# EndlessReform/smoltts

Measured on AMD Instinct MI355X. Metric: Mimi frames/sec (=12.5 x RTF), greedy DualAR decode + Mimi decode to PCM, higher is better.
Workload: dtype bf16 weights, fp32 activations/accumulate, fp32 KV cache (LM); fp32 (Mimi)

## Files before the change

smoltts_amd/csrc/argmax_dev.h:

```cpp
#pragma once
#include "x3.h"

namespace smoltts {

struct Top2 {
  float v1;
  int i1;
  float v2;
};
__device__ __forceinline__ Top2 top2_merge(Top2 a, Top2 b) {
  Top2 o;
  const bool a_first = (a.v1 > b.v1) || (a.v1 == b.v1 && a.i1 < b.i1);
  if (a_first) {
    o.v1 = a.v1; o.i1 = a.i1; o.v2 = fmaxf(a.v2, b.v1);
  } else {
    o.v1 = b.v1; o.i1 = b.i1; o.v2 = fmaxf(b.v2, a.v1);
  }
  return o;
}

__device__ __forceinline__ uint32_t mix32(uint32_t x) {
  x ^= x >> 16; x *= 0x7feb352dU; x ^= x >> 15; x *= 0x846ca68bU; x ^= x >> 16;
  return x;
}
__device__ __forceinline__ float uniform01(uint64_t seed, int slot, int frame, int step, int col) {
  uint32_t h = mix32((uint32_t)seed ^ 0x9E3779B9U * (uint32_t)(slot + 1));
  h = mix32(h ^ (uint32_t)(seed >> 32) ^ 0x85EBCA6BU * (uint32_t)(frame + 1));
  h = mix32(h ^ 0xC2B2AE35U * (uint32_t)(step + 1));
  h = mix32(h ^ 0x27D4EB2FU * (uint32_t)(col + 1));
  return ((float)(h >> 8) + 0.5f) * (1.0f / 16777216.0f);
}

struct ArgmaxScratch {
  Top2 sh[4];
  Top2 sh2[4];
  int id;
};

__device__ __forceinline__ int argmax_row(const float* row, int n_cols, bool ld_vec, int r, float* margin, const int* margin_mask,
                                          const SampleArgs& sa, ArgmaxScratch& S) {
  const int tid = threadIdx.x, lane = tid & 63, wave = tid >> 6;
  float temp = sa.temp, min_p = sa.min_p;
  uint64_t seed = sa.seed;
  int key_slot = r;
  if (sa.table) {
    const SmolttsSlotSampling en = sa.table[r];
    temp = sa.step == 0 ? en.temp : en.fast_temp;
    min_p = temp > 0.f ? en.min_p : 0.f;
    seed = en.seed;
    key_slot = 0;
  }
  Top2 t{-INFINITY, 0x7fffffff, -INFINITY};
#define ST_TAKE(V, J)                                                                               \
  {                                                                                                 \
    const float v_ = (V);                                                                           \
    if (v_ > t.v1) {  \
      t.v2 = t.v1; t.v1 = v_; t.i1 = (J);                                                           \
    } else if (v_ > t.v2) {                                                                         \
      t.v2 = v_;                                                                                    \
    }                                                                                               \
  }
  const bool vec = (n_cols & 3) == 0 && ld_vec && n_cols <= 8 * 1024;
  float4 v[8];
  if (vec) {
#pragma unroll
    for (int i = 0; i < 8; ++i) {
      const int j = tid * 4 + i * 1024;
      v[i] = j < n_cols ? *reinterpret_cast<const float4*>(row + j) : make_float4(-INFINITY, -INFINITY, -INFINITY, -INFINITY);
    }
#pragma unroll
    for (int i = 0; i < 8; ++i) {
      const int j = tid * 4 + i * 1024;
      if (j < n_cols) { ST_TAKE(v[i].x, j) ST_TAKE(v[i].y, j + 1) ST_TAKE(v[i].z, j + 2) ST_TAKE(v[i].w, j + 3) }
    }
  } else {
    for (int j = tid; j < n_cols; j += 256) ST_TAKE(row[j], j)
  }
#undef ST_TAKE
#pragma unroll
  for (int o = 32; o > 0; o >>= 1) {
    Top2 b;
    b.v1 = __shfl_xor(t.v1, o); b.i1 = __shfl_xor(t.i1, o); b.v2 = __shfl_xor(t.v2, o);
    t = top2_merge(t, b);
  }
  if (lane == 0) S.sh[wave] = t;
  __syncthreads();
  Top2 a = top2_merge(top2_merge(S.sh[0], S.sh[1]), top2_merge(S.sh[2], S.sh[3]));
  if (temp > 0.f) {
    const int frame = sa.frames ? sa.frames[r] : sa.frame_base + r;
    if (!sa.table && sa.salt) seed += 0x9E3779B97F4A7C15ULL * (uint64_t)sa.salt[r];
    const float inv_t = 1.0f / temp;
    const float cut = min_p > 0.f ? logf(min_p) : -INFINITY;
    Top2 k{-INFINITY, 0x7fffffff, -INFINITY};
#define ST_KEY(V, J)                                                  \
  {                                                                   \
    const float z = ((V) - a.v1) * inv_t;                   \
    if (z >= cut) {                                                   \
      const float u = uniform01(seed, key_slot, frame, sa.step, (J)); \
      const float key = z - logf(-logf(u));                           \
      if (key > k.v1) { k.v1 = key; k.i1 = (J); }                     \
    }                                                                 \
  }
    if (vec) {
#pragma unroll
      for (int i = 0; i < 8; ++i) {
        const int j = tid * 4 + i * 1024;
        if (j < n_cols) { ST_KEY(v[i].x, j) ST_KEY(v[i].y, j + 1) ST_KEY(v[i].z, j + 2) ST_KEY(v[i].w, j + 3) }
      }
    } else {
      for (int j = tid; j < n_cols; j += 256) ST_KEY(row[j], j)
    }
#undef ST_KEY
#pragma unroll
    for (int o = 32; o > 0; o >>= 1) {
      Top2 b;
      b.v1 = __shfl_xor(k.v1, o); b.i1 = __shfl_xor(k.i1, o); b.v2 = -INFINITY;
      k = top2_merge(k, b);
    }
    if (lane == 0) S.sh2[wave] = k;
    __syncthreads();
    const Top2 w = top2_merge(top2_merge(S.sh2[0], S.sh2[1]), top2_merge(S.sh2[2], S.sh2[3]));
    a.i1 = w.i1;
  }
  if (a.i1 < 0 || a.i1 >= n_cols) a.i1 = 0;
  if (tid == 0) {
    if (temp <= 0.f && margin && (margin_mask == nullptr || margin_mask[r])) {
      const float gap = a.v1 - a.v2;
      if (gap < margin[r]) {
        margin[r] = gap;
        if (sa.margin_at) sa.margin_at[r] = (sa.frames ? sa.frames[r] : sa.frame_base + r) * 64 + sa.step;
      }
    }
  }
  return a.i1;
}

template <int CTRL>
__device__ __forceinline__ Top2 top2_dpp(Top2 t) {
  Top2 b;
  b.v1 = __int_as_float(__builtin_amdgcn_update_dpp(0, __float_as_int(t.v1), CTRL, 0xF, 0xF, true));
  b.i1 = __builtin_amdgcn_update_dpp(0, t.i1, CTRL, 0xF, 0xF, true);
  b.v2 = __int_as_float(__builtin_amdgcn_update_dpp(0, __float_as_int(t.v2), CTRL, 0xF, 0xF, true));
  return top2_merge(t, b);
}
template <bool ROWS32>
__device__ __forceinline__ Top2 top2_swap(Top2 t, int lane) {
  const unsigned a[3] = {__float_as_uint(t.v1), (unsigned)t.i1, __float_as_uint(t.v2)};
  unsigned o[3];
  const bool upper = (lane & (ROWS32 ? 32 : 16)) != 0;
#pragma unroll
  for (int i = 0; i < 3; ++i) {
    if (ROWS32) {
      const auto r = __builtin_amdgcn_permlane32_swap(a[i], a[i], false, false);
      o[i] = upper ? r[0] : r[1];
    } else {
      const auto r = __builtin_amdgcn_permlane16_swap(a[i], a[i], false, false);
      o[i] = upper ? r[0] : r[1];
    }
  }
  return top2_merge(t, Top2{__uint_as_float(o[0]), (int)o[1], __uint_as_float(o[2])});
}
__device__ __forceinline__ Top2 cand_pick_wave(const float* cand, int tiles, int lane) {
  Top2 t{-INFINITY, 0x7fffffff, -INFINITY};
  for (int j = lane; j < tiles; j += 64) {
    const float4 c = *reinterpret_cast<const float4*>(cand + (size_t)j * 4);
    t = top2_merge(t, Top2{c.x, __float_as_int(c.y), c.z});
  }
  t = top2_dpp<0xB1>(t);
  t = top2_dpp<0x4E>(t);
  t = top2_dpp<0x141>(t);
  t = top2_dpp<0x140>(t);
  t = top2_swap<false>(t, lane);
  t = top2_swap<true>(t, lane);
  return t;
}

struct QkvGather {
  const float* table;
  const float* rope;
  float* q_out;
  float* kc;
  float* vc;
  int n_q_heads, n_kv_heads, cache_len, pos;
};

__device__ __forceinline__ float4 rope_gathered4(float4 v, float4 cs) {
#pragma clang fp contract(off)
  const float o0 = v.x * cs.x - v.y * cs.y, o1 = v.y * cs.x + v.x * cs.y;
  const float o2 = v.z * cs.z - v.w * cs.w, o3 = v.w * cs.z + v.z * cs.w;
  return make_float4(o0, o1, o2, o3);
}

constexpr int QG_MAX = 2;
struct QkvRegs { float4 v[QG_MAX], cs[QG_MAX]; };

__device__ __forceinline__ void qkv_gather_load(const QkvGather& g, long erow, int base, QkvRegs& o) {
  const int qd = g.n_q_heads * 64, kd = g.n_kv_heads * 64, nqkv = qd + 2 * kd;
  const float* trow = g.table + erow * nqkv;
#pragma unroll
  for (int i = 0; i < QG_MAX; ++i) {
    const int n0 = base + (threadIdx.x + i * 256) * 4;
    o.v[i] = n0 < nqkv ? *reinterpret_cast<const float4*>(trow + n0) : make_float4(0.f, 0.f, 0.f, 0.f);
    o.cs[i] = n0 < qd + kd ? *reinterpret_cast<const float4*>(g.rope + ((long)g.pos * 32 + ((n0 & 63) >> 1)) * 2) : make_float4(1.f, 0.f, 1.f, 0.f);
  }
}

__device__ __forceinline__ void qkv_gather_store(const QkvGather& g, int r, int base, const QkvRegs& in) {
  const int qd = g.n_q_heads * 64, kd = g.n_kv_heads * 64, nqkv = qd + 2 * kd;
#pragma unroll
  for (int i = 0; i < QG_MAX; ++i) {
    const int n0 = base + (threadIdx.x + i * 256) * 4;
    if (n0 >= nqkv) continue;
    float4 v = in.v[i];
    if (n0 < qd + kd) v = rope_gathered4(v, in.cs[i]);
    if (n0 < qd) {
      *reinterpret_cast<float4*>(g.q_out + (long)r * qd + n0) = v;
    } else {
      const int nn = n0 - qd;
      float* dst = nn < kd ? g.kc : g.vc;
      const int h = (nn < kd ? nn : nn - kd) >> 6, d = nn & 63;
      *reinterpret_cast<float4*>(dst + (((long)r * g.n_kv_heads + h) * g.cache_len + g.pos) * 64 + d) = v;
    }
  }
}

}
```

smoltts_amd/csrc/gemm3.hip:

```cpp
#include <stdlib.h>

#include "argmax_dev.h"
#ifndef SMOLTTS_DBG_PIECES
#define SMOLTTS_DBG_PIECES 3
#endif
#ifndef SMOLTTS_DBG_PIECES_RESID
#define SMOLTTS_DBG_PIECES_RESID SMOLTTS_DBG_PIECES
#endif

namespace smoltts {

struct Gemm3Dev {
  const char* w;
  const float* wscale;
  const char* x3;
  int M, N, K;
  int w_nt;
  int f8_act;
  int half_rows;
  const float* ssq_in;
  float eps;
  const float* bias;
  const float* resid;
  float* out;
// ... 585 lines not shown
  for (int g = 0; g < G; ++g) {
    const float* qp = PICK ? trow + (u.kvc * G + g) * 64 + 4 * m8 : p.aq + (long)row * qd + (u.kvc * G + g) * 64 + 4 * m8;
    u.qa[g] = *reinterpret_cast<const float4*>(qp);
    u.qb[g] = *reinterpret_cast<const float4*>(qp + 32);
  }
  if (PICK) {
    const float4 csa = *reinterpret_cast<const float4*>(p.pk_rope + ((long)p.a_pos * 32 + 2 * m8) * 2);
    const float4 csb = *reinterpret_cast<const float4*>(p.pk_rope + ((long)p.a_pos * 32 + 16 + 2 * m8) * 2);
#pragma unroll
    for (int g = 0; g < G; ++g) { u.qa[g] = rope_gathered4(u.qa[g], csa); u.qb[g] = rope_gathered4(u.qb[g], csb); }
    const float4 ra0 = rope_gathered4(u.ka0, csa), rb0 = rope_gathered4(u.kb0, csb);
    if (new0) { u.ka0 = ra0; u.kb0 = rb0; }
    if (TWO) {
      const float4 ra1 = rope_gathered4(u.ka1, csa), rb1 = rope_gathered4(u.kb1, csb);
      if (new1) { u.ka1 = ra1; u.kb1 = rb1; }
    }
    if (write_kv && u.hv && (new0 || new1)) {
      float* kw = p.kc + cb + (long)p.a_pos * 64;
      float* vw = p.vc + cb + (long)p.a_pos * 64;
      const float4 ka = new0 ? u.ka0 : u.ka1, kb = new0 ? u.kb0 : u.kb1, va = new0 ? u.va0 : u.va1, vb = new0 ? u.vb0 : u.vb1;
      *reinterpret_cast<float4*>(kw) = ka; *reinterpret_cast<float4*>(kw + 32) = kb;
      *reinterpret_cast<float4*>(vw + 32 * hb) = va; *reinterpret_cast<float4*>(vw + 32 * (1 - hb)) = vb;
    }
  }
}

template <int G, bool TWO>
__device__ __forceinline__ void awo_compute(const AwoUnit<G, TWO>& u, char* frag, int lane) {
#pragma clang fp contract(off)
  constexpr int R = AWO_R;
  const int hb = (lane >> 3) & 1, m8 = lane & 7;
  const bool up = (lane & 16) != 0;
#pragma unroll
  for (int g = 0; g < G; ++g) {
    const float4 a = make_float4(u.qa[g].x * 0.125f, u.qa[g].y * 0.125f, u.qa[g].z * 0.125f, u.qa[g].w * 0.125f);
    const float4 b = make_float4(u.qb[g].x * 0.125f, u.qb[g].y * 0.125f, u.qb[g].z * 0.125f, u.qb[g].w * 0.125f);
    float s0 = score16(a, b, u.ka0, u.kb0), s1 = -INFINITY;
    s0 = u.ok0 ? s0 : -INFINITY;
    if (TWO) {
      s1 = score16(a, b, u.ka1, u.kb1);
      s1 = u.ok1 ? s1 : -INFINITY;
    }
    float mx = TWO ? fmaxf(s0, s1) : s0;
    mx = fmaxf(mx, dpp_ror8(mx));
    {
      float t = mx;
      swap16(mx, t);
      mx = fmaxf(mx, t);
    }
    const float e0 = __expf(s0 - mx);
    float den = e0;
    float4 oa = make_float4(e0 * u.va0.x, e0 * u.va0.y, e0 * u.va0.z, e0 * u.va0.w);
    float4 ob = make_float4(e0 * u.vb0.x, e0 * u.vb0.y, e0 * u.vb0.z, e0 * u.vb0.w);
    if (TWO) {
      const float e1 = __expf(s1 - mx);
      den += e1;
      oa.x = fmaf(e1, u.va1.x, oa.x); oa.y = fmaf(e1, u.va1.y, oa.y); oa.z = fmaf(e1, u.va1.z, oa.z); oa.w = fmaf(e1, u.va1.w, oa.w);
      ob.x = fmaf(e1, u.vb1.x, ob.x); ob.y = fmaf(e1, u.vb1.y, ob.y); ob.z = fmaf(e1, u.vb1.z, ob.z); ob.w = fmaf(e1, u.vb1.w, ob.w);
    }
    den += dpp_ror8(den);
    {
      float t = den;
      swap16(den, t);
      den += t;
    }
    oa.x += dpp_ror8(ob.x); oa.y += dpp_ror8(ob.y); oa.z += dpp_ror8(ob.z); oa.w += dpp_ror8(ob.w);
    swap16(oa.x, oa.z);
    swap16(oa.y, oa.w);
    const float inv = 1.0f / den;
    const float ox = (oa.x + oa.z) * inv, oy = (oa.y + oa.w) * inv;
    uint32_t h, mm, l;
    split3_pair(ox, oy, h, mm, l);
    const int c = 2 * (u.kvc * G + g) + hb;
    char* fp = frag + ((size_t)((c * 3) * 4 + (m8 >> 1)) * R + u.rl) * 16 + (m8 & 1) * 8 + (up ? 4 : 0);
    if (u.hv) {
      *reinterpret_cast<uint32_t*>(fp) = h;
      *reinterpret_cast<uint32_t*>(fp + 4 * R * 16) = mm;
      *reinterpret_cast<uint32_t*>(fp + 8 * R * 16) = l;
    }
  }
}

constexpr int AWO_NA = 4, AWO_NB = 8, AWO_U = 3;

template <int G, int T, bool TWO, bool W8, bool PICK, int NBF>
__global__ __launch_bounds__(768) void attn_wo_kernel(const char* w_, const float* kc_, const float* vc_, const float* q_or_cand, const float* pk_table_,
                                                      int m_tiles, int N_, int K_, int heads_pos, Gemm3Dev p) {
  KernargTouch<AWO_KERNARG_LINES> kt;
  kernarg_touch(kt);
  p.w = w_; p.kc = const_cast<float*>(kc_); p.vc = const_cast<float*>(vc_); p.pk_table = pk_table_;
  if (PICK) p.pk_cand = q_or_cand; else p.aq = q_or_cand;
  p.M = m_tiles & 0xffff; p.pk_tiles = m_tiles >> 16; p.N = N_; p.K = K_;
  p.n_q_heads = heads_pos & 255; p.n_kv_heads = (heads_pos >> 8) & 255; p.cache_len = (heads_pos >> 16) & 255; p.a_pos = heads_pos >> 24;
  constexpr int WTILE = W8 ? 512 : 1024, WLANE = W8 ? 8 : 16;
  constexpr int R = AWO_R, NA = AWO_NA, NB = AWO_NB, U = AWO_U;
  extern __shared__ __attribute__((aligned(16))) float smem[];
  const int tid = threadIdx.x, wave = __builtin_amdgcn_readfirstlane(tid >> 6), lane = tid & 63;
  const int r = lane & 15, q = lane >> 4;
  const int ng = blockIdx.x, row0 = blockIdx.y * R;
  const int nchunks = p.K >> 5;
  constexpr bool FULL = NBF != 0;
  const int nb = FULL ? NBF : ((nchunks + 2) / 3 < 1 ? 1 : ((nchunks + 2) / 3 > NB ? NB : (nchunks + 2) / 3));
  char* frag = reinterpret_cast<char*>(smem);
  float4* red4 = reinterpret_cast<float4*>(frag + (size_t)nchunks * 3 * 4 * R * 16);
  STAMP3(0);

  if (wave < NA) {
    const int kv_pairs = (p.n_kv_heads + 1) >> 1;
    const int n_units = (p.M - row0 < R ? p.M - row0 : R) * kv_pairs;
    long erow0 = 0, erow1 = 0;
    Top2 t0{0.f, 0, 0.f}, t1 = t0;
#if SMOLTTS_DBG_AWO_ORDER
    if (PICK) __syncthreads();
#endif
    if (PICK) {
      const int n_cols = p.pk_tiles * 16;
      t0 = cand_pick_wave(p.pk_cand + (size_t)row0 * p.pk_tiles * 4, p.pk_tiles, lane);
      t1 = t0;
      if (row0 + 1 < p.M) t1 = cand_pick_wave(p.pk_cand + (size_t)(row0 + 1) * p.pk_tiles * 4, p.pk_tiles, lane);
      if (t0.i1 < 0 || t0.i1 >= n_cols) t0.i1 = 0;
      if (t1.i1 < 0 || t1.i1 >= n_cols) t1.i1 = 0;
      erow0 = (long)t0.i1 + p.pk_off;
      erow1 = (long)t1.i1 + p.pk_off;
    }
    AwoUnit<G, TWO> un;
    if (wave < n_units) awo_load<G, TWO, PICK>(un, p, wave, kv_pairs, row0, lane, wave / kv_pairs ? erow1 : erow0, blockIdx.x == 0);
    kernarg_touched(kt);
    const bool fin = wave < T;
    const int tf = fin ? wave : 0;
    const int m = row0 + r;
    const bool row_on = r < R;
    const bool mvalid = fin && row_on && m < p.M;
    float4 rr, bb, ga, gb, ws;
    rr = bb = make_float4(0.f, 0.f, 0.f, 0.f);
    ga = gb = ws = make_float4(1.f, 1.f, 1.f, 1.f);
    if (fin) {
      const int mc = m < p.M ? m : p.M - 1;
      const int n0r = (ng * T + tf) * 16 + q * 4;
      const int n0 = n0r < p.N ? n0r : p.N - 4;
      if (W8) ws = *reinterpret_cast<const float4*>(p.wscale + n0);
      if (PICK) {
        const uint2 e = *reinterpret_cast<const uint2*>(p.pk_emb + ((r & 1) ? erow1 : erow0) * p.K + n0);
        rr = make_float4(bf16_lo(e.x), bf16_hi(e.x), bf16_lo(e.y), bf16_hi(e.y));
      } else {
        rr = *reinterpret_cast<const float4*>(p.resid + (long)mc * p.ldo + n0);
      }
      if (p.bias != nullptr) bb = *reinterpret_cast<const float4*>(p.bias + n0);
      if (p.emit.x3a && p.emit.gamma_a) ga = *reinterpret_cast<const float4*>(p.emit.gamma_a + n0);
      if (p.emit.x3b && p.emit.gamma_b) gb = *reinterpret_cast<const float4*>(p.emit.gamma_b + n0);
    }
    STAMP3(5);
#if SMOLTTS_DBG_AWO_ORDER
    if (!PICK) __syncthreads();
#endif
    if (wave < n_units) awo_compute(un, frag, lane);
    for (int unit = wave + NA; unit < n_units; unit += NA) {
      awo_load<G, TWO, PICK>(un, p, unit, kv_pairs, row0, lane, unit / kv_pairs ? erow1 : erow0, blockIdx.x == 0);
      awo_compute(un, frag, lane);
    }
    STAMP3(6);
    __syncthreads();
    __syncthreads();
    STAMP3(3);
    if (PICK && blockIdx.x == 0 && wave == NA - 1 && lane == 0) {
#pragma unroll
      for (int rl = 0; rl < R; ++rl) {
        const int row = row0 + rl;
        if (row >= p.M) break;
        const Top2 t = rl ? t1 : t0;
        p.pk_ids[(long)row * p.pk_ids_stride] = t.i1;
        if (p.pk_margin && (p.pk_mask == nullptr || p.pk_mask[row])) {
          const float gap = t.v1 - t.v2;
          if (gap < p.pk_margin[row]) {
            p.pk_margin[row] = gap;
            if (p.pk_margin_at) p.pk_margin_at[row] = p.pk_frames[row] * 64 + p.pk_step;
          }
        }
      }
    }
    if (!fin) return;
    float4 part[NB];
#pragma unroll
    for (int w = 0; w < NB; ++w) part[w] = red4[((w < nb ? w : 0) * T + tf) * 64 + lane];
    float v[4] = {0.f, 0.f, 0.f, 0.f};
#pragma unroll
    for (int w = 0; w < NB; ++w) {
      const bool on = w < nb;
      v[0] += on ? part[w].x : 0.f;
      v[1] += on ? part[w].y : 0.f;
      v[2] += on ? part[w].z : 0.f;
      v[3] += on ? part[w].w : 0.f;
    }
    const int ntile = ng * T + tf;
    const int n0 = ntile * 16 + q * 4;
    const bool valid = mvalid && n0 < p.N;
    if (W8) { v[0] *= ws.x; v[1] *= ws.y; v[2] *= ws.z; v[3] *= ws.w; }
    v[0] = v[0] + bb.x + rr.x; v[1] = v[1] + bb.y + rr.y; v[2] = v[2] + bb.z + rr.z; v[3] = v[3] + bb.w + rr.w;
    if (valid) {
      *reinterpret_cast<float4*>(p.out + (long)m * p.ldo + n0) = make_float4(v[0], v[1], v[2], v[3]);
      if (p.emit.x3a) x3_emit4(p.emit.x3a, m, n0, p.N >> 5, v[0] * ga.x, v[1] * ga.y, v[2] * ga.z, v[3] * ga.w);
      if (p.emit.x3b) x3_emit4(p.emit.x3b, m, n0, p.N >> 5, v[0] * gb.x, v[1] * gb.y, v[2] * gb.z, v[3] * gb.w);
    }
    if (p.emit.ssq) {
      float sq = valid ? ((v[0] * v[0] + v[1] * v[1]) + (v[2] * v[2] + v[3] * v[3])) : 0.f;
      sq = sum_xor16_32(sq);
      if (q == 0 && mvalid && ntile * 16 < p.N) p.emit.ssq[(size_t)m * (p.N >> 4) + ntile] = sq;
    }
    STAMP3(4);
    return;
// ... 279 lines not shown
```

smoltts_amd/csrc/lm_engine.hip:

```cpp
#include <stdlib.h>
#include <string.h>

#include <new>

#include "argmax_dev.h"
#include "embed_dev.h"

using namespace smoltts;

struct SmolttsEngine {
  SmolttsLMConfig cfg;
  SmolttsLMWeights w;
  const char* arena;
  size_t arena_bytes;
  const float* fast_qkv;
};

constexpr int STAGE_RING = 8;

struct SmolttsSession {
  SmolttsEngine* e;
  int B, max_seq, max_rows, max_frames;
  int stop_on_eos;
  float temp, fast_temp, min_p;
// ... 118 lines not shown
  s->mask = cv.take<int>(B);
  s->iota = cv.take<int>(B);
  s->fastpos = cv.take<int>((size_t)c.n_fast * B);
  s->stage_slots = cv.take<int>(B);
  s->stage_last = cv.take<int>(B);
  s->margin = cv.take<float>(B);
  s->attn_part = cv.take<float>(ATT_SPLIT_PART_FLOATS);
  s->attn_ticket = cv.take<int>(ATT_SPLIT_MAX_PAIRS);
  s->margin_at = cv.take<int>(B);
  s->codes = cv.take<int>(B * (size_t)s->max_frames * H);
  s->slot_tab_area = cv.take<SmolttsSlotSampling>(2 * B + (B * sizeof(int) + sizeof(SmolttsSlotSampling) - 1) / sizeof(SmolttsSlotSampling));
  *total = cv.off;
}

__global__ void init_state_kernel(int B, int n_fast, int* iota, int* fastpos, int* pos, int* frames, int* done, int* mask,
                                  float* margin, int* margin_at, int* cur_col, int* new_col, int* salt, int* attn_ticket) {
  const int b = blockIdx.x * blockDim.x + threadIdx.x;
  for (int i = b; i < ATT_SPLIT_MAX_PAIRS; i += gridDim.x * blockDim.x) attn_ticket[i] = 0;
  if (b >= B) return;
  margin_at[b] = 0;
  iota[b] = b;
  for (int i = 0; i < n_fast; ++i) fastpos[i * B + b] = i;
  pos[b] = 0; frames[b] = 0; done[b] = 1; mask[b] = 0; salt[b] = 0;
  margin[b] = INFINITY;
  for (int i = 0; i <= n_fast; ++i) { cur_col[b * (1 + n_fast) + i] = 0; new_col[b * (1 + n_fast) + i] = 0; }
}

__global__ void slot_sampling_scatter_kernel(int n, const SmolttsSlotSampling* entries, const int* slots, SmolttsSlotSampling* table) {
  const int i = blockIdx.x * blockDim.x + threadIdx.x;
  if (i < n) table[slots[i]] = entries[i];
}

__global__ void slot_reset_kernel(int B, int n_slots, const int* slots, const int* last_row, const int* row_pos, int* pos,
                                  int* frames, int* done, int* mask, float* margin, int* salt) {
  const int b = blockIdx.x * blockDim.x + threadIdx.x;
  if (b >= B) return;
  int hit = -1;
  for (int i = 0; i < n_slots; ++i)
    if (slots[i] == b) hit = i;
  mask[b] = hit >= 0;
  if (hit >= 0) {
    pos[b] = row_pos[last_row[hit]] + 1;
    frames[b] = 0; done[b] = 0; margin[b] = INFINITY;
    salt[b] += 1;
  }
}

__global__ void slot_start_kernel(int B, int H, int n_slots, const int* slots, const int* last_row, const int* row_pos,
                                  const int* grid, int* pos, int* frames, int* done, float* margin, int* cur_col, int* salt) {
  const int b = blockIdx.x * blockDim.x + threadIdx.x;
  if (b >= B) return;
  for (int i = 0; i < n_slots; ++i)
    if (slots[i] == b) {
      const int lr = last_row[i];
      pos[b] = row_pos[lr];
      frames[b] = 0; done[b] = 0; margin[b] = INFINITY;
      salt[b] += 1;
      for (int k = 0; k < H; ++k) cur_col[b * H + k] = grid[(long)lr * H + k];
    }
}

__global__ void slot_park_kernel(int B, int n_slots, const int* slots, const int* last_row, const int* row_pos, int* pos,
                                 int* done, int* mask) {
  const int b = blockIdx.x * blockDim.x + threadIdx.x;
  if (b >= B) return;
  for (int i = 0; i < n_slots; ++i)
    if (slots[i] == b) { pos[b] = row_pos[last_row[i]] + 1; done[b] = 1; mask[b] = 0; }
}

__global__ void slot_parkpos_kernel(int B, int n_slots, const int* slots, const int* where, int* pos, int* done, int* mask) {
  const int b = blockIdx.x * blockDim.x + threadIdx.x;
  if (b >= B) return;
  for (int i = 0; i < n_slots; ++i)
    if (slots[i] == b) { pos[b] = where[i]; done[b] = 1; mask[b] = 0; }
}

struct CommitArgs {
  int B, H, max_frames, max_seq, im_end, stop_on_eos, advance_pos, do_commit;
  int* new_col;
  int *mask, *cur_col, *codes, *pos, *frames, *done;
  const float* slow_logits; int slow_cols; SampleArgs slow_sa;
  const float* last_logits; int last_cols; SampleArgs last_sa;
  float* margin;
  const float* slow_cand; int slow_tiles;
  const float* last_cand; int last_tiles;
  int* attn_ticket;
};

__global__ __launch_bounds__(256) void commit_embed_kernel(CommitArgs a, EmbedTables t, float* xt, EmitDev emit) {
  __shared__ int s_col[64];
  __shared__ float sh4[4];
  __shared__ ArgmaxScratch s_pick[2];
  const int b = blockIdx.x, tid = threadIdx.x, H = a.H;
  if (b == 0 && a.attn_ticket)
    for (int i = tid; i < ATT_SPLIT_MAX_PAIRS; i += blockDim.x) a.attn_ticket[i] = 0;
  int id_slow = 0, id_last = 0;
  const bool c_slow = a.slow_logits && a.slow_cand, c_last = a.last_logits && a.last_cand;
  if (c_slow || c_last) {
    __shared__ int s_id[2];
    __shared__ float s_gap[2];
    const int wave = tid >> 6, lane = tid & 63;
    if ((wave == 0 && c_slow) || (wave == 1 && c_last)) {
      const float* cand = wave == 0 ? a.slow_cand + (size_t)b * a.slow_tiles * 4 : a.last_cand + (size_t)b * a.last_tiles * 4;
      Top2 t = cand_pick_wave(cand, wave == 0 ? a.slow_tiles : a.last_tiles, lane);
      if (t.i1 < 0 || t.i1 >= (wave == 0 ? a.slow_cols : a.last_cols)) t.i1 = 0;
      if (lane == 0) { s_id[wave] = t.i1; s_gap[wave] = t.v1 - t.v2; }
    }
    __syncthreads();
    if (tid == 0 && a.margin && a.mask[b]) {
#pragma unroll
      for (int k = 0; k < 2; ++k) {
        if (!(k == 0 ? c_slow : c_last)) continue;
        const SampleArgs& sa = k == 0 ? a.slow_sa : a.last_sa;
        if (s_gap[k] < a.margin[b]) {
          a.margin[b] = s_gap[k];
          if (sa.margin_at) sa.margin_at[b] = (sa.frames ? sa.frames[b] : sa.frame_base + b) * 64 + sa.step;
        }
      }
    }
    if (c_slow) id_slow = s_id[0];
    if (c_last) id_last = s_id[1];
  }
  if (a.slow_logits && !c_slow) id_slow = argmax_row(a.slow_logits + (long)b * a.slow_cols, a.slow_cols, (a.slow_cols & 3) == 0, b, a.margin, a.mask, a.slow_sa, s_pick[0]);
  if (a.last_logits && !c_last) id_last = argmax_row(a.last_logits + (long)b * a.last_cols, a.last_cols, (a.last_cols & 3) == 0, b, a.margin, a.mask, a.last_sa, s_pick[1]);
  int f = 0;
  bool live = false;
  if (tid < 64) { f = a.frames[b]; live = a.do_commit && a.mask[b]; }
  const bool publish = live && f < a.max_frames;
  int slow_now = 0;
  if (tid < H) {
    int nv = a.new_col[b * H + tid];
    if (a.slow_logits && tid == 0) nv = id_slow;
    if (a.last_logits && tid == H - 1) nv = id_last;
    if ((a.slow_logits && tid == 0) || (a.last_logits && tid == H - 1)) a.new_col[b * H + tid] = nv;
    const int v = publish ? nv : a.cur_col[b * H + tid];
    s_col[tid] = v;
    if (publish) {
      a.cur_col[b * H + tid] = v;
      a.codes[((long)b * a.max_frames + f) * H + tid] = v;
    }
  }
  slow_now = a.slow_logits ? id_slow : a.new_col[b * H];
  if (tid == 0) {
    int d = a.done[b];
    if (live) {
      int p = a.pos[b];
      if (a.advance_pos) a.pos[b] = ++p;
      if (publish) a.frames[b] = f + 1;
      if ((a.stop_on_eos && slow_now == a.im_end) || f + 1 >= a.max_frames || p >= a.max_seq) a.done[b] = d = 1;
    }
    a.mask[b] = !d;
  }
  __syncthreads();
  embed_row(t, s_col, b, xt, emit, sh4);
}

SmolttsGemm3Args base3(int fmt, const void* w, const void* x3, int M, int N, int K, int epilogue) {
  SmolttsGemm3Args a;
  memset(&a, 0, sizeof(a));
  a.w_dev = w; a.x3_dev = x3; a.M = M; a.N = N; a.K = K; a.epilogue = epilogue;
  a.w_format = fmt;
  if (fmt == SMOLTTS_W_FP8) a.w_scale_dev = reinterpret_cast<const float*>(static_cast<const char*>(w) + (size_t)N * K);
  return a;
}

bool dup_hit(const SmolttsSession* s, int code, int N) { return s->dup_code == code && (s->dup_n <= 0 || s->dup_n == N); }

int launch_gemm3_m(const SmolttsSession* s, const SmolttsGemm3Args& a, hipStream_t st) {
  ST_TRY(launch_gemm3(a, st));
  if (a.epilogue != SMOLTTS_EPI_RESID && dup_hit(s, a.epilogue, a.N)) ST_TRY(launch_gemm3(a, st));
  return SMOLTTS_OK;
}

int run_block(const SmolttsSession* s, const SmolttsBlockWeights& bw, int dim, int n_head, int n_kv, int inter, float* x,
              float* q, int M, const int* row_pos, const int* row_slot, const float* rope, void* kc, void* vc,
              int cache_len, const char* in_x3, const EmitArgs& next, hipStream_t st, bool first_pos = false,
              int kv_format = SMOLTTS_KV_F32, int iota_pos = -1, bool qkv_done = false, int w_stream = 0,
              const SmolttsPickArgs* pick = nullptr) {
  const SmolttsEngine* e = s->e;
  const char* A = e->arena;
  const float eps = e->cfg.norm_eps;
  if (!qkv_done) {
    SmolttsGemm3Args a = base3(e->cfg.weight_format, A + bw.wqkv, in_x3, M, (n_head + 2 * n_kv) * 64, dim, SMOLTTS_EPI_QKV_ROPE);
    a.fp8_activations = s->fp8_prefill;
    a.ssq_in_dev = s->ssq; a.eps = eps; a.out_dev = q; a.ldo = n_head * 64;
    a.rope_dev = rope; a.row_pos_dev = row_pos; a.row_slot_dev = row_slot;
    a.k_cache_dev = (float*)kc; a.v_cache_dev = (float*)vc; a.n_q_heads = n_head; a.n_kv_heads = n_kv; a.cache_len = cache_len;
    a.kv_format = kv_format; a.w_stream = (w_stream & (1 | SMOLTTS_STREAM_W_DEPTH_QKVO)) != 0;
    if (first_pos) a.v_x3_dev = s->x3a;
    ST_TRY(launch_gemm3_m(s, a, st));
  }
  const bool fused_attn = !first_pos && iota_pos > 0 && s->fuse_depth_attn && kv_format == SMOLTTS_KV_F32 &&
                          smoltts_gemm3_attn_fusable(n_head, n_kv, cache_len) && dim == n_head * 64;
  if (!first_pos && !fused_attn) {
    const int reps = dup_hit(s, cache_len <= 16 ? 100 : 101, 0) ? 2 : 1;
    for (int i = 0; i < reps; ++i)
      ST_TRY(launch_attention(q, kc, vc, row_pos, row_slot, M, n_head, n_kv, cache_len, 0, nullptr, s->x3a, st, kv_format, iota_pos,
                              s->split_attn ? s->attn_part : nullptr, s->attn_ticket));
  }
  {
    SmolttsGemm3Args a = base3(e->cfg.weight_format, A + bw.wo, s->x3a, M, dim, dim, SMOLTTS_EPI_RESID);
    a.fp8_activations = s->fp8_prefill;
    a.resid_dev = x; a.out_dev = x; a.ldo = dim;
    a.emit_a_dev = s->x3n; a.gamma_a_dev = (const float*)(A + bw.ffn_norm); a.ssq_out_dev = s->ssq; a.w_stream = (w_stream & (1 | SMOLTTS_STREAM_W_DEPTH_QKVO)) != 0;
    if (fused_attn) {
      a.attn_q_dev = q; a.attn_pos = iota_pos; a.k_cache_dev = (float*)kc; a.v_cache_dev = (float*)vc;
      a.n_q_heads = n_head; a.n_kv_heads = n_kv; a.cache_len = cache_len; a.kv_format = SMOLTTS_KV_F32;
      a.pick = pick;
    }
    ST_REQUIRE(pick == nullptr || fused_attn, SMOLTTS_E_STATE, "run_block: a pick needs the fused depth attention");
    ST_TRY(launch_gemm3(a, st));
  }
  {
    SmolttsGemm3Args a = base3(e->cfg.weight_format, A + bw.w13, s->x3n, M, 2 * inter, dim, SMOLTTS_EPI_SWIGLU);
    a.fp8_activations = s->fp8_prefill;
    a.ssq_in_dev = s->ssq; a.eps = eps; a.x3_out_dev = s->x3h; a.w_stream = (w_stream & (1 | SMOLTTS_STREAM_W_DEPTH_W13)) != 0;
    ST_TRY(launch_gemm3_m(s, a, st));
  }
  {
    SmolttsGemm3Args a = base3(e->cfg.weight_format, A + bw.w2, s->x3h, M, dim, inter, SMOLTTS_EPI_RESID);
    a.fp8_activations = s->fp8_prefill;
    a.resid_dev = x; a.out_dev = x; a.ldo = dim;
    a.emit_a_dev = next.x3a; a.gamma_a_dev = next.gamma_a; a.emit_b_dev = next.x3b; a.gamma_b_dev = next.gamma_b;
    a.ssq_out_dev = next.ssq; a.w_stream = (w_stream & (1 | SMOLTTS_STREAM_W_DEPTH_W2)) != 0;
    ST_TRY(launch_gemm3(a, st));
  }
  return SMOLTTS_OK;
}

const float* gamma_at(const SmolttsEngine* e, uint64_t off) { return (const float*)(e->arena + off); }

EmitArgs slow_hidden_emit(const SmolttsSession* s) {
  const SmolttsEngine* e = s->e;
  EmitArgs em{s->x3n, gamma_at(e, e->w.norm), s->x3n2,
              e->cfg.has_fast_project_in ? nullptr : gamma_at(e, e->w.fast_layers[0].attn_norm), s->ssq};
  return em;
}

__global__ __launch_bounds__(256) void scatter_last_kernel(const float* xr, const int* slots, const int* last_row, int dim,
                                                           float* xt) {
  const int i = blockIdx.x;
  const long src = last_row[i], dst = slots[i];
  for (int d = threadIdx.x * 4; d < dim; d += 256 * 4)
    *reinterpret_cast<float4*>(xt + dst * dim + d) = *reinterpret_cast<const float4*>(xr + src * dim + d);
}

EmbedTables embed_tables(const SmolttsEngine* e) {
  const SmolttsLMConfig& c = e->cfg;
  const char* A = e->arena;
  return EmbedTables{(const uint16_t*)(A + e->w.text_emb), (const uint16_t*)(A + e->w.codebook_emb), c.dim, c.codebook_size,
                     c.duplicate_code_0 ? 0 : c.codebook_size, c.embed_mask_mode, c.semantic_start_id, c.semantic_end_id,
                     c.vocab_size, c.codebook_size * c.num_codebooks, c.n_fast};
}

bool slow_sampled(const SmolttsSession* s) { return s->slot_mode ? (s->form & 1) != 0 : s->temp > 0.f; }
bool fast_sampled(const SmolttsSession* s) { return s->slot_mode ? (s->form & 2) != 0 : s->fast_temp > 0.f; }

SampleArgs pick_args(const SmolttsSession* s, int step) {
  if (s->slot_mode) {
    const bool sampled = step == 0 ? slow_sampled(s) : fast_sampled(s);
    return SampleArgs{0.f, 0.f, 0, step, 0, s->frames, nullptr, s->margin_at, sampled ? s->slot_tab : nullptr};
  }
  if (step == 0) return SampleArgs{s->temp, s->min_p, s->seed, 0, 0, s->frames, s->salt, s->margin_at, nullptr};
  return SampleArgs{s->fast_temp, s->fast_temp > 0.f ? s->min_p : 0.f, s->seed, step, 0, s->frames, s->salt, s->margin_at, nullptr};
}

bool commit_cand_slow(const SmolttsSession* s) { return s->commit_picks && s->fuse_pick && !slow_sampled(s) && s->B < 256; }
bool commit_cand_last(const SmolttsSession* s) { return s->commit_picks && s->fuse_pick && !fast_sampled(s) && s->B < 256; }

int launch_commit_embed(SmolttsSession* s, int do_commit, int advance_pos, hipStream_t st, bool picks = false) {
  const SmolttsEngine* e = s->e;
  const SmolttsLMConfig& c = e->cfg;
  ST_REQUIRE(1 + c.n_fast <= 64 && c.dim % 64 == 0, SMOLTTS_E_INVALID, "commit: grid height > 64 or dim %% 64 != 0");
  CommitArgs a;
  memset(&a, 0, sizeof(a));
  a.B = s->B; a.H = 1 + c.n_fast; a.max_frames = s->max_frames; a.max_seq = s->max_seq; a.im_end = c.im_end_id;
  a.stop_on_eos = s->stop_on_eos; a.advance_pos = advance_pos; a.do_commit = do_commit;
  a.new_col = s->new_col; a.mask = s->mask; a.cur_col = s->cur_col; a.codes = s->codes; a.pos = s->pos; a.frames = s->frames; a.done = s->done;
  a.margin = s->margin;
  a.attn_ticket = s->attn_ticket;
  if (picks) {
    a.slow_logits = s->logits_slow; a.slow_cols = c.vocab_size;
    a.slow_sa = pick_args(s, 0);
    a.last_logits = s->logits; a.last_cols = c.codebook_size;
    a.last_sa = pick_args(s, c.n_fast);
    if (commit_cand_slow(s)) { a.slow_cand = s->cand_slow; a.slow_tiles = (c.vocab_size + 15) / 16; }
    if (commit_cand_last(s)) { a.last_cand = s->cand; a.last_tiles = (c.codebook_size + 15) / 16; }
  }
  const EmitDev em{s->x3n, gamma_at(e, e->w.layers[0].attn_norm), nullptr, nullptr, s->ssq};
  hipLaunchKernelGGL(commit_embed_kernel, dim3(s->B), dim3(256), 0, st, a, embed_tables(e), s->xt, em);
  ST_CHECK_HIP(hipGetLastError());
  return SMOLTTS_OK;
}

int run_tail(SmolttsSession* s, int advance_pos, hipStream_t st) {
  const SmolttsEngine* e = s->e;
  const SmolttsLMConfig& c = e->cfg;
  const char* A = e->arena;
  const int B = s->B, H = 1 + c.n_fast;
  {
    SmolttsGemm3Args a = base3(c.weight_format, A + e->w.head, s->x3n, B, c.vocab_size, c.dim, SMOLTTS_EPI_STORE);
    a.ssq_in_dev = s->ssq; a.eps = c.norm_eps; a.out_dev = s->logits_slow; a.ldo = c.vocab_size; a.w_stream = (s->stream_w & SMOLTTS_STREAM_W_SLOW_HEAD) != 0;
    if (commit_cand_slow(s)) a.cand_out_dev = s->cand_slow;
    ST_TRY(launch_gemm3_m(s, a, st));
  }
  const bool picks = s->commit_picks;
  if (!picks) {
    const SampleArgs slow_sa = pick_args(s, 0);
    ST_TRY(launch_argmax(s->logits_slow, B, c.vocab_size, c.vocab_size, s->new_col, H, s->margin, s->mask, nullptr, 0, 0, nullptr,
                         nullptr, &slow_sa, st));
  }
  float* xf = s->xt;
  const char* first_x3 = s->x3n2;
  const EmitArgs to_fast0{s->x3n, gamma_at(e, e->w.fast_layers[0].attn_norm), nullptr, nullptr, s->ssq};
  if (c.has_fast_project_in) {
    SmolttsGemm3Args a = base3(c.weight_format, A + e->w.fast_proj_w, s->x3n2, B, c.fast_dim, c.dim, SMOLTTS_EPI_STORE);
    a.bias_dev = (const float*)(A + e->w.fast_proj_b); a.out_dev = s->xf; a.ldo = c.fast_dim;
    a.emit_a_dev = to_fast0.x3a; a.gamma_a_dev = to_fast0.gamma_a; a.ssq_out_dev = s->ssq;
    ST_TRY(launch_gemm3(a, st));
    xf = s->xf;
    first_x3 = s->x3n;
  }
  const size_t fl_stride = (size_t)B * c.fast_n_kv_head * c.n_fast * 64;
  const bool table = e->fast_qkv != nullptr && s->use_qkv_table;
  const bool pick_fused = s->fuse_pick && table && s->fuse_depth_attn && !fast_sampled(s) && B < 256 && c.codebook_size % 16 == 0 &&
                          c.fast_dim == c.fast_n_head * 64 && smoltts_gemm3_attn_fusable(c.fast_n_head, c.fast_n_kv_head, c.n_fast);
  SmolttsPickArgs pk;
  memset(&pk, 0, sizeof(pk));
  bool pk_pending = false;
  for (int i = 0; i < c.n_fast; ++i) {
    for (int l = 0; l < c.n_fast_layer; ++l) {
      const EmitArgs next{s->x3n,
                          gamma_at(e, l + 1 < c.n_fast_layer ? e->w.fast_layers[l + 1].attn_norm : e->w.fast_norm),
                          nullptr, nullptr, s->ssq};
      ST_TRY(run_block(s, e->w.fast_layers[l], c.fast_dim, c.fast_n_head, c.fast_n_kv_head, c.fast_inter, xf, s->qt, B,
                       s->fastpos + (size_t)i * B, s->iota, (const float*)(A + e->w.fast_rope), s->fkc + l * fl_stride,
                       s->fvc + l * fl_stride, c.n_fast, (i == 0 && l == 0) ? first_x3 : s->x3n, next, st, i == 0,
                       SMOLTTS_KV_F32, i, table && i > 0 && l == 0,
                       s->stream_w & (SMOLTTS_STREAM_W_DEPTH_QKVO | SMOLTTS_STREAM_W_DEPTH_W13 | SMOLTTS_STREAM_W_DEPTH_W2),
                       (pk_pending && l == 0) ? &pk : nullptr));
      if (l == 0) pk_pending = false;
    }
    {
      const size_t wrow = (size_t)i * e->w.fast_head_step_stride;
      const size_t wbytes = c.weight_format == SMOLTTS_W_FP8 ? wrow * (c.fast_dim + 4) : wrow * c.fast_dim * 2;
      SmolttsGemm3Args a = base3(c.weight_format, A + e->w.fast_head + wbytes, s->x3n, B, c.codebook_size, c.fast_dim, SMOLTTS_EPI_STORE);
      a.ssq_in_dev = s->ssq; a.eps = c.norm_eps; a.out_dev = s->logits; a.ldo = c.codebook_size;
      a.w_stream = (s->stream_w & SMOLTTS_STREAM_W_DEPTH_HEAD) != 0;
      if (pick_fused && i + 1 < c.n_fast) a.cand_out_dev = s->cand;
      if (i + 1 == c.n_fast && commit_cand_last(s)) a.cand_out_dev = s->cand;
      ST_TRY(launch_gemm3_m(s, a, st));
    }
    const SampleArgs fast_sa = pick_args(s, 1 + i);
    if (i + 1 == c.n_fast) {
      if (!picks)
        ST_TRY(launch_argmax(s->logits, B, c.codebook_size, c.codebook_size, s->new_col + 1 + i, H, s->margin, s->mask, nullptr, 0, 0,
                             nullptr, nullptr, &fast_sa, st));
      break;
    }
    const int off = c.depthwise_wte ? (c.duplicate_code_0 ? i : i + 1) * c.codebook_size : 0;
    float* xnext = c.has_fast_project_in ? s->xf : s->xt;
    if (pick_fused) {
      pk.cand_dev = s->cand; pk.cand_tiles = c.codebook_size / 16; pk.qkv_table_dev = e->fast_qkv;
      pk.rope_dev = (const float*)(A + e->w.fast_rope); pk.emb_dev = A + e->w.fast_emb; pk.emb_row_offset = off;
      pk.ids_dev = s->new_col + 1 + i; pk.ids_stride = H; pk.margin_dev = s->margin; pk.margin_mask_dev = s->mask;
      pk.margin_at_dev = s->margin_at; pk.frames_dev = s->frames; pk.step = 1 + i;
      pk_pending = true;
      xf = xnext;
      continue;
    }
    QkvGather qg;
    memset(&qg, 0, sizeof(qg));
    if (table)
// ... 668 lines not shown
```

smoltts_amd/csrc/x3.h:

```cpp
#pragma once
#include "common.h"

namespace smoltts {

typedef __bf16 bf16x2_t __attribute__((ext_vector_type(2)));
typedef __bf16 bf16x8_t __attribute__((ext_vector_type(8)));

__device__ __forceinline__ uint32_t pack_bf16(float a, float b) {
  bf16x2_t h = {(__bf16)a, (__bf16)b};
  return __builtin_bit_cast(uint32_t, h);
}

__device__ __forceinline__ void split3_pair(float a, float b, uint32_t& h, uint32_t& m, uint32_t& l) {
  h = pack_bf16(a, b);
  const float ra = a - bf16_lo(h), rb = b - bf16_hi(h);
  m = pack_bf16(ra, rb);
  l = pack_bf16(ra - bf16_lo(m), rb - bf16_hi(m));
}

__device__ __forceinline__ size_t x3_offset(int m, int k, int nchunks) {
  const int mtile = m >> 4, r = m & 15, c = k >> 5, q = (k & 31) >> 3, j0 = k & 7;
  return ((size_t)mtile * nchunks + c) * 3072 + (size_t)(q * 16 + r) * 16 + j0 * 2;
}

__device__ __forceinline__ void x3_emit4(char* x3, int m, int k, int nchunks, float a0, float a1, float a2, float a3) {
  uint32_t h0, m0, l0, h1, m1, l1;
  split3_pair(a0, a1, h0, m0, l0);
  split3_pair(a2, a3, h1, m1, l1);
  char* p = x3 + x3_offset(m, k, nchunks);
  *reinterpret_cast<uint2*>(p) = make_uint2(h0, h1);
  *reinterpret_cast<uint2*>(p + 1024) = make_uint2(m0, m1);
  *reinterpret_cast<uint2*>(p + 2048) = make_uint2(l0, l1);
}

__device__ __forceinline__ void x3_emit2(char* x3, int m, int k, int nchunks, float a0, float a1) {
  uint32_t h, mm, l;
  split3_pair(a0, a1, h, mm, l);
  char* p = x3 + x3_offset(m, k, nchunks);
  *reinterpret_cast<uint32_t*>(p) = h;
  *reinterpret_cast<uint32_t*>(p + 1024) = mm;
  *reinterpret_cast<uint32_t*>(p + 2048) = l;
}

struct EmitDev {
  char* x3a;
  const float* gamma_a;
  char* x3b;
  const float* gamma_b;
  float* ssq;
};

__device__ __forceinline__ void emit_x4(const EmitDev& e, int m, int k, int nchunks, float x0, float x1, float x2, float x3v) {
  if (e.x3a) {
    if (e.gamma_a) {
      const float4 g = *reinterpret_cast<const float4*>(e.gamma_a + k);
      x3_emit4(e.x3a, m, k, nchunks, x0 * g.x, x1 * g.y, x2 * g.z, x3v * g.w);
    } else {
      x3_emit4(e.x3a, m, k, nchunks, x0, x1, x2, x3v);
    }
  }
  if (e.x3b) {
    if (e.gamma_b) {
      const float4 g = *reinterpret_cast<const float4*>(e.gamma_b + k);
      x3_emit4(e.x3b, m, k, nchunks, x0 * g.x, x1 * g.y, x2 * g.z, x3v * g.w);
    } else {
      x3_emit4(e.x3b, m, k, nchunks, x0, x1, x2, x3v);
    }
  }
}

__device__ __forceinline__ void emit_row_ssq(const EmitDev& e, int m, int dim, float local_ss, float* sh4) {
  if (!e.ssq) return;
  const int lane = threadIdx.x & 63, wave = threadIdx.x >> 6;
  float s = local_ss;
#pragma unroll
  for (int o = 32; o > 0; o >>= 1) s += __shfl_xor(s, o);
  if (lane == 0) sh4[wave] = s;
  __syncthreads();
  const int nt = dim >> 4;
  for (int i = threadIdx.x; i < nt; i += blockDim.x)
    e.ssq[(size_t)m * nt + i] = i == 0 ? ((sh4[0] + sh4[1]) + sh4[2]) + sh4[3] : 0.f;
}

}
```

Measured before the change: 28650.

## Batch candidate loads, overlap pick with attention load, specialize commit kernel

Candidate top-2 picks now load all tiles into registers with unrolled, predicated loads instead of a strided loop. In the attention+wo kernel, each wave computes its own row's pick first and issues its weight/KV load before merging the other row, so the load overlaps the second merge. The commit kernel is templated on whether row argmax is needed and takes candidate pointers as direct kernargs with prefetch, moving the ticket reset after the pick. It also switches shuffles to a lane_xor_c helper and makes top2_merge branch-free. The changes add code size and template variants.

```diff
diff --git a/smoltts_amd/csrc/argmax_dev.h b/smoltts_amd/csrc/argmax_dev.h
--- a/smoltts_amd/csrc/argmax_dev.h
+++ b/smoltts_amd/csrc/argmax_dev.h
@@ -1,5 +1,9 @@
 #pragma once
 #include "x3.h"
+
+#ifndef SMOLTTS_OPT_PICK_LOADS
+#define SMOLTTS_OPT_PICK_LOADS 1
+#endif
 
 namespace smoltts {
 
@@ -9,14 +13,9 @@
   float v2;
 };
 __device__ __forceinline__ Top2 top2_merge(Top2 a, Top2 b) {
-  Top2 o;
-  const bool a_first = (a.v1 > b.v1) || (a.v1 == b.v1 && a.i1 < b.i1);
-  if (a_first) {
-    o.v1 = a.v1; o.i1 = a.i1; o.v2 = fmaxf(a.v2, b.v1);
-  } else {
-    o.v1 = b.v1; o.i1 = b.i1; o.v2 = fmaxf(b.v2, a.v1);
-  }
-  return o;
+  const bool a_first = (a.v1 > b.v1) | ((a.v1 == b.v1) & (a.i1 < b.i1));
+  const float va2 = fmaxf(a.v2, b.v1), vb2 = fmaxf(b.v2, a.v1);
+  return Top2{a_first ? a.v1 : b.v1, a_first ? a.i1 : b.i1, a_first ? va2 : vb2};
 }
 
 __device__ __forceinline__ uint32_t mix32(uint32_t x) {
@@ -80,7 +79,7 @@
 #pragma unroll
   for (int o = 32; o > 0; o >>= 1) {
     Top2 b;
-    b.v1 = __shfl_xor(t.v1, o); b.i1 = __shfl_xor(t.i1, o); b.v2 = __shfl_xor(t.v2, o);
+    b.v1 = lane_xor_c(t.v1, o, lane); b.i1 = __float_as_int(lane_xor_c(__int_as_float(t.i1), o, lane)); b.v2 = lane_xor_c(t.v2, o, lane);
     t = top2_merge(t, b);
   }
   if (lane == 0) S.sh[wave] = t;
@@ -114,7 +113,7 @@
 #pragma unroll
     for (int o = 32; o > 0; o >>= 1) {
       Top2 b;
-      b.v1 = __shfl_xor(k.v1, o); b.i1 = __shfl_xor(k.i1, o); b.v2 = -INFINITY;
+      b.v1 = lane_xor_c(k.v1, o, lane); b.i1 = __float_as_int(lane_xor_c(__int_as_float(k.i1), o, lane)); b.v2 = -INFINITY;
       k = top2_merge(k, b);
     }
     if (lane == 0) S.sh2[wave] = k;
@@ -160,12 +159,7 @@
   }
   return top2_merge(t, Top2{__uint_as_float(o[0]), (int)o[1], __uint_as_float(o[2])});
 }
-__device__ __forceinline__ Top2 cand_pick_wave(const float* cand, int tiles, int lane) {
-  Top2 t{-INFINITY, 0x7fffffff, -INFINITY};
-  for (int j = lane; j < tiles; j += 64) {
-    const float4 c = *reinterpret_cast<const float4*>(cand + (size_t)j * 4);
-    t = top2_merge(t, Top2{c.x, __float_as_int(c.y), c.z});
-  }
+__device__ __forceinline__ Top2 top2_ladder(Top2 t, int lane) {
   t = top2_dpp<0xB1>(t);
   t = top2_dpp<0x4E>(t);
   t = top2_dpp<0x141>(t);
@@ -173,6 +167,55 @@
   t = top2_swap<false>(t, lane);
   t = top2_swap<true>(t, lane);
   return t;
+}
+__device__ __forceinline__ Top2 cand_pick_wave(const float* cand, int tiles, int lane) {
+  Top2 t{-INFINITY, 0x7fffffff, -INFINITY};
+  for (int j = lane; j < tiles; j += 64) {
+    const float4 c = *reinterpret_cast<const float4*>(cand + (size_t)j * 4);
+    t = top2_merge(t, Top2{c.x, __float_as_int(c.y), c.z});
+  }
+  return top2_ladder(t, lane);
+}
+
+template <int N>
+struct CandRegs {
+  float4 c[N];
+};
+template <int N>
+__device__ __forceinline__ void cand_load(const float* cand, int tiles, int lane, CandRegs<N>& o) {
+#pragma unroll
+  for (int i = 0; i < N; ++i) {
+    const int j = lane + 64 * i;
+    o.c[i] = *reinterpret_cast<const float4*>(cand + (size_t)(j < tiles ? j : tiles - 1) * 4);
+  }
+}
+template <int N>
+__device__ __forceinline__ Top2 cand_merge(const CandRegs<N>& in, int tiles, int lane) {
+  Top2 t{-INFINITY, 0x7fffffff, -INFINITY};
+#pragma unroll
+  for (int i = 0; i < N; ++i) {
+    const Top2 m = top2_merge(t, Top2{in.c[i].x, __float_as_int(in.c[i].y), in.c[i].z});
+    const bool on = lane + 64 * i < tiles;
+    t.v1 = on ? m.v1 : t.v1;
+    t.i1 = on ? m.i1 : t.i1;
+    t.v2 = on ? m.v2 : t.v2;
+  }
+  return top2_ladder(t, lane);
+}
+template <int N>
+__device__ __forceinline__ Top2 cand_pick_wave_n(const float* cand, int tiles, int lane) {
+  CandRegs<N> r;
+  cand_load<N>(cand, tiles, lane, r);
+  return cand_merge<N>(r, tiles, lane);
+}
+__device__ __forceinline__ Top2 cand_pick_wave_lf(const float* cand, int tiles, int lane) {
+  switch ((tiles + 63) >> 6) {
+    case 1: return cand_pick_wave_n<1>(cand, tiles, lane);
+    case 2: return cand_pick_wave_n<2>(cand, tiles, lane);
+    case 3: return cand_pick_wave_n<3>(cand, tiles, lane);
+    case 4: return cand_pick_wave_n<4>(cand, tiles, lane);
+    default: return cand_pick_wave(cand, tiles, lane);
+  }
 }
 
 struct QkvGather {
diff --git a/smoltts_amd/csrc/gemm3.hip b/smoltts_amd/csrc/gemm3.hip
--- a/smoltts_amd/csrc/gemm3.hip
+++ b/smoltts_amd/csrc/gemm3.hip
@@ -691,6 +691,7 @@
 }
 
 constexpr int AWO_NA = 4, AWO_NB = 8, AWO_U = 3;
+constexpr int AWO_PICK_N = 2;
 
 template <int G, int T, bool TWO, bool W8, bool PICK, int NBF>
 __global__ __launch_bounds__(768) void attn_wo_kernel(const char* w_, const float* kc_, const float* vc_, const float* q_or_cand, const float* pk_table_,
@@ -719,21 +720,44 @@
     const int n_units = (p.M - row0 < R ? p.M - row0 : R) * kv_pairs;
     long erow0 = 0, erow1 = 0;
     Top2 t0{0.f, 0, 0.f}, t1 = t0;
+    AwoUnit<G, TWO> un;
+    bool loaded = false;
 #if SMOLTTS_DBG_AWO_ORDER
     if (PICK) __syncthreads();
 #endif
     if (PICK) {
       const int n_cols = p.pk_tiles * 16;
-      t0 = cand_pick_wave(p.pk_cand + (size_t)row0 * p.pk_tiles * 4, p.pk_tiles, lane);
-      t1 = t0;
-      if (row0 + 1 < p.M) t1 = cand_pick_wave(p.pk_cand + (size_t)(row0 + 1) * p.pk_tiles * 4, p.pk_tiles, lane);
-      if (t0.i1 < 0 || t0.i1 >= n_cols) t0.i1 = 0;
-      if (t1.i1 < 0 || t1.i1 >= n_cols) t1.i1 = 0;
+#if SMOLTTS_OPT_PICK_LOADS
+      if (p.pk_tiles <= 64 * AWO_PICK_N) {
+        const int own = wave < n_units ? wave / kv_pairs : 0;
+        const float* c0 = p.pk_cand + (size_t)row0 * p.pk_tiles * 4;
+        const float* c1 = row0 + 1 < p.M ? c0 + (size_t)p.pk_tiles * 4 : c0;
+        CandRegs<AWO_PICK_N> ca, cb;
+        cand_load<AWO_PICK_N>(own ? c1 : c0, p.pk_tiles, lane, ca);
+        cand_load<AWO_PICK_N>(own ? c0 : c1, p.pk_tiles, lane, cb);
+        Top2 ta = cand_merge<AWO_PICK_N>(ca, p.pk_tiles, lane);
+        if (ta.i1 < 0 || ta.i1 >= n_cols) ta.i1 = 0;
+        if (wave < n_units) {
+          awo_load<G, TWO, PICK>(un, p, wave, kv_pairs, row0, lane, (long)ta.i1 + p.pk_off, blockIdx.x == 0);
+          loaded = true;
+        }
+        Top2 tb = cand_merge<AWO_PICK_N>(cb, p.pk_tiles, lane);
+        if (tb.i1 < 0 || tb.i1 >= n_cols) tb.i1 = 0;
+        t0 = own ? tb : ta;
+        t1 = own ? ta : tb;
+      } else
+#endif
+      {
+        t0 = cand_pick_wave(p.pk_cand + (size_t)row0 * p.pk_tiles * 4, p.pk_tiles, lane);
+        t1 = t0;
+        if (row0 + 1 < p.M) t1 = cand_pick_wave(p.pk_cand + (size_t)(row0 + 1) * p.pk_tiles * 4, p.pk_tiles, lane);
+        if (t0.i1 < 0 || t0.i1 >= n_cols) t0.i1 = 0;
+        if (t1.i1 < 0 || t1.i1 >= n_cols) t1.i1 = 0;
+      }
       erow0 = (long)t0.i1 + p.pk_off;
       erow1 = (long)t1.i1 + p.pk_off;
     }
-    AwoUnit<G, TWO> un;
-    if (wave < n_units) awo_load<G, TWO, PICK>(un, p, wave, kv_pairs, row0, lane, wave / kv_pairs ? erow1 : erow0, blockIdx.x == 0);
+    if (wave < n_units && !loaded) awo_load<G, TWO, PICK>(un, p, wave, kv_pairs, row0, lane, wave / kv_pairs ? erow1 : erow0, blockIdx.x == 0);
     kernarg_touched(kt);
     const bool fin = wave < T;
     const int tf = fin ? wave : 0;
diff --git a/smoltts_amd/csrc/lm_engine.hip b/smoltts_amd/csrc/lm_engine.hip
--- a/smoltts_amd/csrc/lm_engine.hip
+++ b/smoltts_amd/csrc/lm_engine.hip
@@ -224,27 +224,37 @@
   const float* slow_logits; int slow_cols; SampleArgs slow_sa;
   const float* last_logits; int last_cols; SampleArgs last_sa;
   float* margin;
-  const float* slow_cand; int slow_tiles;
-  const float* last_cand; int last_tiles;
   int* attn_ticket;
 };
 
-__global__ __launch_bounds__(256) void commit_embed_kernel(CommitArgs a, EmbedTables t, float* xt, EmitDev emit) {
+struct CommitKernargs {
+  const float* slow_cand; const float* last_cand; int slow_tiles, last_tiles;
+  CommitArgs a; EmbedTables t; float* xt; EmitDev emit;
+};
+constexpr int COMMIT_KERNARG_LINES = ((int)sizeof(CommitKernargs) - 1) / 64;
+
+template <bool ROWS>
+__global__ __launch_bounds__(256) void commit_embed_kernel(const float* slow_cand, const float* last_cand, int slow_tiles, int last_tiles,
+                                                           CommitArgs a, EmbedTables t, float* xt, EmitDev emit) {
+  KernargTouch<COMMIT_KERNARG_LINES> kt;
+  kernarg_touch(kt);
   __shared__ int s_col[64];
   __shared__ float sh4[4];
   __shared__ ArgmaxScratch s_pick[2];
   const int b = blockIdx.x, tid = threadIdx.x, H = a.H;
-  if (b == 0 && a.attn_ticket)
-    for (int i = tid; i < ATT_SPLIT_MAX_PAIRS; i += blockDim.x) a.attn_ticket[i] = 0;
   int id_slow = 0, id_last = 0;
-  const bool c_slow = a.slow_logits && a.slow_cand, c_last = a.last_logits && a.last_cand;
+  const bool c_slow = slow_cand != nullptr, c_last = last_cand != nullptr;
   if (c_slow || c_last) {
     __shared__ int s_id[2];
     __shared__ float s_gap[2];
-    const int wave = tid >> 6, lane = tid & 63;
+    const int wave = __builtin_amdgcn_readfirstlane(tid >> 6), lane = tid & 63;
     if ((wave == 0 && c_slow) || (wave == 1 && c_last)) {
-      const float* cand = wave == 0 ? a.slow_cand + (size_t)b * a.slow_tiles * 4 : a.last_cand + (size_t)b * a.last_tiles * 4;
-      Top2 t = cand_pick_wave(cand, wave == 0 ? a.slow_tiles : a.last_tiles, lane);
+      const float* cand = wave == 0 ? slow_cand + (size_t)b * slow_tiles * 4 : last_cand + (size_t)b * last_tiles * 4;
+#if SMOLTTS_OPT_PICK_LOADS
+      Top2 t = cand_pick_wave_lf(cand, wave == 0 ? slow_tiles : last_tiles, lane);
+#else
+      Top2 t = cand_pick_wave(cand, wave == 0 ? slow_tiles : last_tiles, lane);
+#endif
       if (t.i1 < 0 || t.i1 >= (wave == 0 ? a.slow_cols : a.last_cols)) t.i1 = 0;
       if (lane == 0) { s_id[wave] = t.i1; s_gap[wave] = t.v1 - t.v2; }
     }
@@ -263,8 +273,11 @@
     if (c_slow) id_slow = s_id[0];
     if (c_last) id_last = s_id[1];
   }
-  if (a.slow_logits && !c_slow) id_slow = argmax_row(a.slow_logits + (long)b * a.slow_cols, a.slow_cols, (a.slow_cols & 3) == 0, b, a.margin, a.mask, a.slow_sa, s_pick[0]);
-  if (a.last_logits && !c_last) id_last = argmax_row(a.last_logits + (long)b * a.last_cols, a.last_cols, (a.last_cols & 3) == 0, b, a.margin, a.mask, a.last_sa, s_pick[1]);
+  if (b == 0 && a.attn_ticket)
+    for (int i = tid; i < ATT_SPLIT_MAX_PAIRS; i += blockDim.x) a.attn_ticket[i] = 0;
+  kernarg_touched(kt);
+  if (ROWS && a.slow_logits && !c_slow) id_slow = argmax_row(a.slow_logits + (long)b * a.slow_cols, a.slow_cols, (a.slow_cols & 3) == 0, b, a.margin, a.mask, a.slow_sa, s_pick[0]);
+  if (ROWS && a.last_logits && !c_last) id_last = argmax_row(a.last_logits + (long)b * a.last_cols, a.last_cols, (a.last_cols & 3) == 0, b, a.margin, a.mask, a.last_sa, s_pick[1]);
   int f = 0;
   bool live = false;
   if (tid < 64) { f = a.frames[b]; live = a.do_commit && a.mask[b]; }
@@ -416,6 +429,8 @@
   ST_REQUIRE(1 + c.n_fast <= 64 && c.dim % 64 == 0, SMOLTTS_E_INVALID, "commit: grid height > 64 or dim %% 64 != 0");
   CommitArgs a;
   memset(&a, 0, sizeof(a));
+  const float *slow_cand = nullptr, *last_cand = nullptr;
+  int slow_tiles = 0, last_tiles = 0;
   a.B = s->B; a.H = 1 + c.n_fast; a.max_frames = s->max_frames; a.max_seq = s->max_seq; a.im_end = c.im_end_id;
   a.stop_on_eos = s->stop_on_eos; a.advance_pos = advance_pos; a.do_commit = do_commit;
   a.new_col = s->new_col; a.mask = s->mask; a.cur_col = s->cur_col; a.codes = s->codes; a.pos = s->pos; a.frames = s->frames; a.done = s->done;
@@ -426,11 +441,17 @@
     a.slow_sa = pick_args(s, 0);
     a.last_logits = s->logits; a.last_cols = c.codebook_size;
     a.last_sa = pick_args(s, c.n_fast);
-    if (commit_cand_slow(s)) { a.slow_cand = s->cand_slow; a.slow_tiles = (c.vocab_size + 15) / 16; }
-    if (commit_cand_last(s)) { a.last_cand = s->cand; a.last_tiles = (c.codebook_size + 15) / 16; }
+    if (commit_cand_slow(s)) { slow_cand = s->cand_slow; slow_tiles = (c.vocab_size + 15) / 16; }
+    if (commit_cand_last(s)) { last_cand = s->cand; last_tiles = (c.codebook_size + 15) / 16; }
   }
   const EmitDev em{s->x3n, gamma_at(e, e->w.layers[0].attn_norm), nullptr, nullptr, s->ssq};
-  hipLaunchKernelGGL(commit_embed_kernel, dim3(s->B), dim3(256), 0, st, a, embed_tables(e), s->xt, em);
+  const bool rows = (a.slow_logits && !slow_cand) || (a.last_logits && !last_cand);
+  if (rows)
+    hipLaunchKernelGGL(commit_embed_kernel<true>, dim3(s->B), dim3(256), 0, st, slow_cand, last_cand, slow_tiles, last_tiles, a,
+                       embed_tables(e), s->xt, em);
+  else
+    hipLaunchKernelGGL(commit_embed_kernel<false>, dim3(s->B), dim3(256), 0, st, slow_cand, last_cand, slow_tiles, last_tiles, a,
+                       embed_tables(e), s->xt, em);
   ST_CHECK_HIP(hipGetLastError());
   return SMOLTTS_OK;
 }
diff --git a/smoltts_amd/csrc/x3.h b/smoltts_amd/csrc/x3.h
--- a/smoltts_amd/csrc/x3.h
+++ b/smoltts_amd/csrc/x3.h
@@ -74,7 +74,7 @@
   const int lane = threadIdx.x & 63, wave = threadIdx.x >> 6;
   float s = local_ss;
 #pragma unroll
-  for (int o = 32; o > 0; o >>= 1) s += __shfl_xor(s, o);
+  for (int o = 32; o > 0; o >>= 1) s += lane_xor_c(s, o, lane);
   if (lane == 0) sh4[wave] = s;
   __syncthreads();
   const int nt = dim >> 4;
```

New measurement: 28940, median of 6. 1.01x the previous value.
